# sshaoshuai/PointRCNN

Hardware: AMD Instinct MI355X
Metric: KITTI frames/sec, RPN inference end-to-end (16384 pts/frame, bs32 per GPU) (higher is better)
Workload: dtype f32 via split-bf16x6 MFMA (every fp32 operand cut exactly into 3 bf16 pieces, 6 bf16 MFMA products per fp32 product, fp32 accumulate: fp32-grade, measured error 2.9e-7 of sum|x||w| vs 3.0e-7 for the fp32-MFMA kernel; hoisted grouped layers on the split kernel too, unhoisted grouped first layers (xyz; 1 GPU; Full RPN PointNet++ backbone (4 SA-MSG + 4 FP) + cls/reg heads, tools/cfgs/default.yaml, 16384 pts/frame, batch 32 per GPU, random-init weights, eval-mode BN; frames_per_gpu=32, npoints=16384, parallelism=frames sharded, dp1, launch=hipGraph replay, streams=20, hw_queues=4, proposal_layer=normal, clouds=uniform, group_dedup=True, roi_dedup=True

## Files before the change

### include/prcnn_pointops.h

```cpp
#ifndef PRCNN_POINTOPS_H
#define PRCNN_POINTOPS_H

#include <stddef.h>
#include <stdint.h>

#ifdef __cplusplus
extern "C" {
#endif

typedef void* prcnn_stream_t;

#define PRCNN_OK 0
#define PRCNN_EINVAL (-1)
#define PRCNN_EHIP (-2)
#define PRCNN_EUNSUPPORTED (-3)

int prcnn_abi_version(void);
const char* prcnn_last_error(void);
const char* prcnn_build_id(void);


int prcnn_fps(const float* xyz, int B, int N, int npoint, float* tmp, int32_t* idx, prcnn_stream_t stream);

int prcnn_fps_status(void);
// ... 34 lines not shown
                       float* out, prcnn_stream_t stream);
int prcnn_three_interp_grad(const float* grad_out, const int32_t* idx, const float* weight, int B, int C, int n,
                            int m, float* grad_feat, float* workspace, prcnn_stream_t stream);


size_t prcnn_wpack_floats(int Nout, int K);
int prcnn_pack_weight(const float* w, int Nout, int K, int k_rot, float* wpack, prcnn_stream_t stream);

int prcnn_mlp_rows(const float* in, int ld_in, int64_t rows, int K, const float* wpack, const float* bias, int Nout,
                   int relu, float* out, int ld_out, int col_off, int pool_ns, const int32_t* rows_dev, int rows_unit,
                   const int32_t* seg_cnt, int seg_rows, prcnn_stream_t stream);

int prcnn_mlp_group(const float* xyz, const float* new_xyz, const int32_t* idx, const float* feat_cl, int ld_feat,
                    int B, int N, int M, int nsample, int C, const float* act_wx, const float* act_bias,
                    const float* wpack, const float* bias, int Nout, int relu, float* out, int ld_out, int col_off,
                    int pool_ns, const int32_t* groups_dev, prcnn_stream_t stream);

int prcnn_mlp_interp(const float* known_cl, int ld_known, const int32_t* idx3, const float* w3, const float* skip_cl,
                     int ld_skip, int B, int n, int m, int C2, int C1, const float* act_bias, const float* wpack,
                     const float* bias, int Nout, int relu, float* out, int ld_out, int col_off,
                     prcnn_stream_t stream);

int prcnn_mlp_rows_addinterp(const float* in, int ld_in, int K, const float* wpack, const float* bias, int Nout,
                             int relu, const float* y_cl, int ld_y, const int32_t* idx3, const float* w3, int B, int n,
                             int m, float* out, int ld_out, int col_off, prcnn_stream_t stream);

size_t prcnn_wsplit_bytes(int Nout, int K);
int prcnn_pack_weight_split(const float* w, int Nout, int K, int chain, void* wsplit, prcnn_stream_t stream);
int prcnn_mlp_rows_split(const float* in, int ld_in, int64_t rows, int K, const float* wpack, const void* wsplit, int terms,
                         const float* bias, int Nout, int relu, float* out, int ld_out, int col_off, int pool_ns,
                         const int32_t* rows_dev, int rows_unit, const int32_t* seg_cnt, int seg_rows, prcnn_stream_t stream);
int prcnn_mlp_chain_rows_split(const float* in, int ld_in, int64_t rows, int K, const void* const* wchain, const float* const* wpack,
                               const float* const* bias, const int* nout, const int* relu, int terms, float* out, int ld_out,
                               int col_off, prcnn_stream_t stream);
int prcnn_mlp_chain_interp_split(const float* known_cl, int ld_known, const int32_t* idx3, const float* w3, int B, int n, int m,
                                 int C2, const float* act_bias, const void* wchain, const float* wpack, const float* bias, int Nout,
                                 int relu, int terms, float* out, int ld_out, int col_off, prcnn_stream_t stream);
int prcnn_mlp_rows_addinterp_split(const float* in, int ld_in, int K, const float* wpack, const void* wsplit, int terms,
                                   const float* bias, int Nout, int relu, const float* y_cl, int ld_y, const int32_t* idx3,
                                   const float* w3, int B, int n, int m, float* out, int ld_out, int col_off,
                                   prcnn_stream_t stream);
int prcnn_mlp_group_split(const float* xyz, const float* new_xyz, const int32_t* idx, const float* feat_cl, int ld_feat, int B, int N,
                          int M, int nsample, int C, const float* act_wx, const float* act_bias, const float* wpack,
                          const void* wsplit, int terms, const float* bias, int Nout, int relu, float* out, int ld_out, int col_off,
                          int pool_ns, const int32_t* groups_dev, prcnn_stream_t stream);

int prcnn_mlp_chain_supported(int mode, int nlayers, const int* nout, int pool_ns);
int prcnn_mlp_chain_rows(const float* in, int ld_in, int64_t rows, int K, int nlayers, const float* const* wpack,
                         const float* const* bias, const int* nout, const int* relu, float* out, int ld_out,
                         int col_off, int pool_ns, const int32_t* seg_cnt, int seg_rows, prcnn_stream_t stream);
int prcnn_mlp_chain_group(const float* xyz, const float* new_xyz, const int32_t* idx, const float* feat_cl,
                          int ld_feat, int B, int N, int M, int nsample, int C, const float* act_wx,
                          const float* act_bias, int nlayers,
                          const float* const* wpack, const float* const* bias, const int* nout, const int* relu,
                          float* out, int ld_out, int col_off, int pool_ns, const int32_t* groups_dev, prcnn_stream_t stream);
int prcnn_mlp_chain_interp(const float* known_cl, int ld_known, const int32_t* idx3, const float* w3,
                           const float* skip_cl, int ld_skip, int B, int n, int m, int C2, int C1,
                           const float* act_bias, int nlayers, const float* const* wpack, const float* const* bias, const int* nout, const int* relu,
                           float* out, int ld_out, int col_off, prcnn_stream_t stream);

int prcnn_maxpool_rows(const float* in, int ld_in, int64_t rows_out, int ns, int C, float* out, int ld_out,
                       int col_off, prcnn_stream_t stream);

int prcnn_roipool3d(const float* xyz, const float* boxes3d, const float* feat, int B, int N, int M, int C, int S,
                    float* pooled, int32_t* empty, prcnn_stream_t stream);
size_t prcnn_roipool3d_work_bytes(int B, int N);
int prcnn_roipool3d_ws(const float* xyz, const float* boxes3d, const float* feat, int B, int N, int M, int C, int S, float* pooled,
                       int32_t* empty, void* work, size_t work_bytes, prcnn_stream_t stream);

int prcnn_pts_in_boxes3d(const float* pts, const float* boxes3d, int N, int M, int32_t* flags, prcnn_stream_t stream);
// ... 134 lines not shown
```

### pointrcnn_amd/_cabi.py

```python
import ctypes
import os

from . import build as _build

_P = ctypes.c_void_p
_I = ctypes.c_int
_F = ctypes.c_float
_L = ctypes.c_int64
_Z = ctypes.c_size_t
_D = ctypes.c_double



class TrainSrc(ctypes.Structure):
    _fields_ = [("mode", _I), ("rows", _L), ("K", _I),
                ("in_", _P), ("ld_in", _I), ("pro_scale", _P), ("pro_shift", _P),
                ("xyz", _P), ("new_xyz", _P), ("idx", _P), ("feat", _P), ("ld_feat", _I),
                ("B", _I), ("N", _I), ("M", _I), ("ns", _I), ("C", _I),
                ("known", _P), ("idx3", _P), ("w3", _P), ("skip", _P), ("ld_known", _I), ("ld_skip", _I),
                ("n", _I), ("m", _I), ("C2", _I), ("C1", _I),
                ("mult", _P), ("rows_dev", _P), ("norm_rows", _L), ("seg_off", _P), ("seg_cnt", _P), ("row_grp", _P), ("groups", _I)]


class TrainLayer(ctypes.Structure):
    _fields_ = [("Nout", _I), ("W", _P), ("gamma", _P), ("beta", _P), ("eps", _F), ("momentum", _F),
                ("running_mean", _P), ("running_var", _P), ("y", _P), ("cst", _P), ("ld_c", _I), ("wpack", _P), ("wpack_t", _P),
                ("dW", _P), ("dgamma", _P), ("dbeta", _P)]


REQUIRED_ABI = 9

SIGNATURES = {
    "prcnn_abi_version": (_I, []),
    "prcnn_last_error": (ctypes.c_char_p, []),
    "prcnn_build_id": (ctypes.c_char_p, []),
    "prcnn_fps": (_I, [_P, _I, _I, _I, _P, _P, _P]),
    "prcnn_fps_status": (_I, []),
    "prcnn_fps_order": (_I, [_P, _I, _I, _I, _I, _P, _P, _P]),
    "prcnn_fps_mode": (_I, [_P, _I, _I, _I, _I, _I, _P, _P, _P]),
    "prcnn_ball_query_arith": (_I, [_P, _P, _I, _I, _I, _F, _I, _I, _P, _P]),
    "prcnn_three_nn_arith": (_I, [_P, _P, _I, _I, _I, _I, _P, _P, _P]),
    "prcnn_rpn_labels": (_I, [_P, _P, _P, _I, _I, _I, _F, _P, _P, _P]),
    "prcnn_gt_aug_edit": (_I, [_P, _P, _P, _P, _P, _F, _P, _P, _P, _I, _I, _I, _I, _P, _P, _P, _P, _P]),
    "prcnn_host_pts_in_boxes3d": (_I, [_P, _P, _L, _L, _P]),
    "prcnn_host_roipool3d": (_I, [_P, _P, _P, _L, _L, _L, _L, _P, _P, _P]),
    "prcnn_gather": (_I, [_P, _P, _I, _I, _I, _I, _P, _P]),
    "prcnn_gather_grad": (_I, [_P, _P, _I, _I, _I, _I, _P, _P]),
    "prcnn_gather_rows": (_I, [_P, _I, _P, _I, _I, _I, _I, _P, _P]),
    "prcnn_ball_query": (_I, [_P, _P, _I, _I, _I, _F, _I, _P, _P]),
    "prcnn_ball_query2": (_I, [_P, _P, _I, _I, _I, _F, _I, _P, _F, _I, _P, _P]),
    "prcnn_group": (_I, [_P, _P, _I, _I, _I, _I, _I, _P, _P]),
    "prcnn_group_grad": (_I, [_P, _P, _I, _I, _I, _I, _I, _P, _P]),
    "prcnn_three_nn": (_I, [_P, _P, _I, _I, _I, _P, _P, _P, _P]),
    "prcnn_three_interp": (_I, [_P, _P, _P, _I, _I, _I, _I, _P, _P]),
    "prcnn_three_interp_grad": (_I, [_P, _P, _P, _I, _I, _I, _I, _P, _P, _P]),
    "prcnn_wpack_floats": (_Z, [_I, _I]),
    "prcnn_pack_weight": (_I, [_P, _I, _I, _I, _P, _P]),
    "prcnn_mlp_rows": (_I, [_P, _I, _L, _I, _P, _P, _I, _I, _P, _I, _I, _I, _P, _I, _P, _I, _P]),
    "prcnn_mlp_group": (_I, [_P, _P, _P, _P, _I, _I, _I, _I, _I, _I, _P, _P, _P, _P, _I, _I, _P, _I, _I, _I, _P, _P]),
    "prcnn_mlp_group_split": (_I, [_P, _P, _P, _P, _I, _I, _I, _I, _I, _I, _P, _P, _P, _P, _I, _P, _I, _I, _P, _I, _I, _I, _P, _P]),
    "prcnn_mlp_interp": (_I, [_P, _I, _P, _P, _P, _I, _I, _I, _I, _I, _I, _P, _P, _P, _I, _I, _P, _I, _I, _P]),
    "prcnn_mlp_rows_addinterp": (_I, [_P, _I, _I, _P, _P, _I, _I, _P, _I, _P, _P, _I, _I, _I, _P, _I, _I, _P]),
    "prcnn_wsplit_bytes": (_Z, [_I, _I]),
    "prcnn_pack_weight_split": (_I, [_P, _I, _I, _I, _P, _P]),
    "prcnn_mlp_chain_interp_split": (_I, [_P, _I, _P, _P, _I, _I, _I, _I, _P, _P, _P, _P, _I, _I, _I, _P, _I, _I, _P]),
    "prcnn_mlp_chain_rows_split": (_I, [_P, _I, _L, _I, _P, _P, _P, _P, _P, _I, _P, _I, _I, _P]),
    "prcnn_mlp_rows_split": (_I, [_P, _I, _L, _I, _P, _P, _I, _P, _I, _I, _P, _I, _I, _I, _P, _I, _P, _I, _P]),
    "prcnn_mlp_rows_addinterp_split": (_I, [_P, _I, _I, _P, _P, _I, _P, _I, _I, _P, _I, _P, _P, _I, _I, _I, _P, _I, _I, _P]),
    "prcnn_mlp_chain_supported": (_I, [_I, _I, _P, _I]),
    "prcnn_mlp_chain_rows": (_I, [_P, _I, _L, _I, _I, _P, _P, _P, _P, _P, _I, _I, _I, _P, _I, _P]),
    "prcnn_mlp_chain_group": (_I, [_P, _P, _P, _P, _I, _I, _I, _I, _I, _I, _P, _P, _I, _P, _P, _P, _P, _P, _I, _I, _I, _P, _P]),
    "prcnn_mlp_chain_interp": (_I, [_P, _I, _P, _P, _P, _I, _I, _I, _I, _I, _I, _P, _I, _P, _P, _P, _P, _P, _I, _I, _P]),
    "prcnn_maxpool_rows": (_I, [_P, _I, _L, _I, _I, _P, _I, _I, _P]),
    "prcnn_roipool3d": (_I, [_P, _P, _P, _I, _I, _I, _I, _I, _P, _P, _P]),
    "prcnn_roipool3d_work_bytes": (_Z, [_I, _I]),
    "prcnn_roipool3d_ws": (_I, [_P, _P, _P, _I, _I, _I, _I, _I, _P, _P, _P, _Z, _P]),
    "prcnn_pts_in_boxes3d": (_I, [_P, _P, _I, _I, _P, _P]),
    "prcnn_boxes_overlap_bev": (_I, [_P, _I, _P, _I, _P, _P]),
    "prcnn_boxes_iou_bev": (_I, [_P, _I, _P, _I, _P, _P]),
    "prcnn_nms_workspace_bytes": (_Z, [_I]),
    "prcnn_nms": (_I, [_P, _I, _F, _I, _I, _P, _P, _P, _Z, _P]),
    "prcnn_decode_bbox_target": (_I, [_P, _I, _P, ctypes.c_long, _I, _D, _D, _I, _P, _I, _I, _D, _D, _I, _I, _P, _P]),
    "prcnn_proposal_workspace_bytes": (_Z, [_I, _I, _I, _I]),
    "prcnn_proposal_layer": (_I, [_P, _P, _I, _I, _I, _F, _F, _F, _I, _I, _I, _I, _F, _I, _P, _P, _P, _P, _Z, _P]),
    "prcnn_nms_batched_workspace_bytes": (_Z, [_I, _I]),
    "prcnn_roipool3d_canonical": (_I, [_P, _P, _P, _P, _P, _P, _I, _I, _I, _I, _I, _I, _P, _I, _P, _I, _P, _P, _P]),
    "prcnn_roipool3d_canonical_ws": (_I, [_P, _P, _P, _P, _P, _P, _I, _I, _I, _I, _I, _I, _P, _I, _P, _I, _P, _P, _P, _Z, _P]),
    "prcnn_grid_bytes": (_Z, [_I, _I]),
    "prcnn_grid_build": (_I, [_P, _I, _I, _F, _I, _P, _Z, _P]),
    "prcnn_ball_query2_grid": (_I, [_P, _P, _P, _I, _I, _I, _F, _I, _P, _F, _I, _P, _P]),
    "prcnn_three_nn_grid": (_I, [_P, _P, _I, _I, _I, _P, _P, _P, _P]),
    "prcnn_rotate_iou_eval": (_I, [_P, _I, _P, _I, _I, _P, _P]),
    "prcnn_kitti_overlaps": (_I, [_I, _P, _P, _P, _P, _P, _I, _P, _P]),
    "prcnn_kitti_statistics": (_I, [_P, _P, _P, _P, _P, _P, _P, _P, _P, _P, _I, _I, _I, _D, _P, _I, _I, _I, _P, _P, _P]),
    "prcnn_group_compact": (_I, [_P, _P, _I, _I, _I, _I, _I, _P, _P, _P, _P, _P, _P, _P, _P, _P, _P, _P]),
    "prcnn_segmax_scatter": (_I, [_P, _I, _P, _P, _P, _P, _I, _I, _P, _I, _I, _P]),
    "prcnn_scatter_rows": (_I, [_P, _I, _P, _P, _I, _I, _P, _I, _I, _P]),
    "prcnn_scene_workspace_bytes": (_Z, [_L, _I]),
    "prcnn_scene_prepare": (_I, [_P, _P, _I, _L, _I, _P, _P, _P, _I, ctypes.c_uint32, _P, _P, _P, _P, _P, _P, _Z, _P]),
# ... 73 lines not shown
```

### pointrcnn_amd/csrc/cabi_common.hip

```cpp
#include "common.h"
#include <stdarg.h>

static thread_local char g_err[512] = "";

int prcnn_fail(int code, const char* fmt, ...) {
    va_list ap;
    va_start(ap, fmt);
    vsnprintf(g_err, sizeof(g_err), fmt, ap);
    va_end(ap);
    return code;
}

PRCNN_API const char* prcnn_last_error(void) { return g_err; }
PRCNN_API int prcnn_abi_version(void) { return 9; }

#ifndef PRCNN_BUILD_ID
#define PRCNN_BUILD_ID "PRCNN_BUILD_ID=unknown"
#endif
PRCNN_API const char* prcnn_build_id(void) { return &PRCNN_BUILD_ID[sizeof("PRCNN_BUILD_ID=") - 1]; }
```

### pointrcnn_amd/csrc/mlp.hip

```cpp
#include "common.h"
#include <stdlib.h>

#define MLP_BM 128
#define MLP_BN 64
#define MLP_BK 32
#define MLP_THREADS 256
#define MLP_ALD 36

typedef float f32x16 __attribute__((ext_vector_type(16)));

enum { MODE_PLAIN = 0, MODE_GROUP = 1, MODE_INTERP = 2 };

struct MlpParams {
    long rows;
    int K, KB, NB;
    const float* wpack;
    const float* bias;
    int Nout, relu;
    float* out;
    int ld_out, col_off, pool_ns;
    const float* in;
    int ld_in;
    const float* xyz;
    const float* new_xyz;
// ... 980 lines not shown
        bool bad = wave_has_nonfinite<2 * WNB>(reinterpret_cast<const f32x16 (&)[2 * WNB]>(acc));
        if (ADDY && addy_done) bad = __syncthreads_or(bad) != 0;
        if (bad && n_active) split_redo_f32<MODE, WNB>(P, acc, row0, wm, wn, nb0, lane);
        if (bad) addy_done = false;
    }
    layer_epilogue<MODE, WNB, ADDY>(P, acc, reinterpret_cast<float*>(Ls), nullptr, tid, row0, nb0, n_active, addy_done);
}

template <int MODE, int WNB, int TERMS, bool ADDY, bool LOOP>
__global__ __launch_bounds__(MLP_THREADS, 2) void mlp_layer_s_kernel(const MlpParams Pin) {
    MlpParams P = Pin;
    P.rows = effective_rows(Pin);
    __shared__ __attribute__((aligned(16))) unsigned char Ls[2 * 3 * SPL_PLANE];
    if constexpr (LOOP) {
        const long nbid = ((P.rows + MLP_BM - 1) / MLP_BM + 7) / 8 * 8 * P.wgm_cols;
        for (long bid = blockIdx.x; bid < nbid; bid += gridDim.x) {
            int tid;
            asm volatile("v_mov_b32 %0, %1" : "=v"(tid) : "v"(threadIdx.x));
            layer_s_tile<MODE, WNB, TERMS, ADDY>(P, bid, 0, tid, Ls);
            __syncthreads();
        }
    } else {
        layer_s_tile<MODE, WNB, TERMS, ADDY>(P, blockIdx.x, blockIdx.y, threadIdx.x, Ls);
    }
}

struct ChainParams {
    MlpParams a;
    const float* wpack1; const float* bias1; int KB1, N1, relu1;
    const float* wpack2; const float* bias2; int KB2, N2, relu2;
    int nlayers;
    int stack_split;
    const void* wsplit1;
};

#define CH_DPP_FMAX(v, ctrl) asm volatile("s_nop 1\n\tv_max_f32_dpp %0, %0, %0 " ctrl : "+v"(v))
#define CH_DPP_FMAX4(v, ctrl)                                                                                   \
    asm volatile("s_nop 1\n\tv_max_f32_dpp %0, %0, %0 " ctrl "\n\tv_max_f32_dpp %1, %1, %1 " ctrl               \
                 "\n\tv_max_f32_dpp %2, %2, %2 " ctrl "\n\tv_max_f32_dpp %3, %3, %3 " ctrl                       \
                 : "+v"(v[0]), "+v"(v[1]), "+v"(v[2]), "+v"(v[3]))

__device__ __forceinline__ float4 ldw(const float* __restrict__ wpack, int KB, int ob, int kb, int lane) {
    return ld4(wpack + (((long)ob * KB + kb) * 64 + lane) * 4);
}

template <int NB>
__device__ __forceinline__ void bias_act(f32x16 (&acc)[NB], const float* __restrict__ bias, int relu, int h) {
#pragma unroll
    for (int ob = 0; ob < NB; ob++)
#pragma unroll
        for (int q = 0; q < 4; q++) {
            float4 b = bias ? ld4(bias + ob * 32 + 8 * q + 4 * h) : make_float4(0.f, 0.f, 0.f, 0.f);
            float v0 = acc[ob][4 * q + 0] + b.x, v1 = acc[ob][4 * q + 1] + b.y;
            float v2 = acc[ob][4 * q + 2] + b.z, v3 = acc[ob][4 * q + 3] + b.w;
            if (relu) { v0 = fmaxf(v0, 0.f); v1 = fmaxf(v1, 0.f); v2 = fmaxf(v2, 0.f); v3 = fmaxf(v3, 0.f); }
            acc[ob][4 * q + 0] = v0; acc[ob][4 * q + 1] = v1; acc[ob][4 * q + 2] = v2; acc[ob][4 * q + 3] = v3;
        }
}

#define CH_WAVES 4
#define CH_STAGE_TILES 16
template <int NB> struct ChStage { static constexpr int G = CH_STAGE_TILES / NB; static constexpr int TPW = (G * NB + CH_WAVES - 1) / CH_WAVES; };

template <int NB>
__device__ __forceinline__ void stage_load(const float* __restrict__ wpack, int KB, int st, int wave, int lane, float4 (&r)[4]) {
    constexpr int G = ChStage<NB>::G;
// ... 830 lines not shown
        mt.w0[u] = w[0]; mt.w1[u] = w[1]; mt.w2[u] = w[2];
    }
}
__device__ __forceinline__ void coop_rows32(const MlpParams& P, long rw0, int g, int q, const CoopMeta<MODE_PLAIN>&, CoopRows32<MODE_PLAIN>& cr) {
#pragma unroll
    for (int u = 0; u < 4; u++) cr.o[u] = (unsigned)(min(rw0 + 8 * u + g, P.rows - 1) * (long)P.ld_in) + 4u * q;
}
__device__ __forceinline__ void coop_rows32(const MlpParams& P, long rw0, int g, int q, const CoopMeta<MODE_INTERP>& mt, CoopRows32<MODE_INTERP>& cr) {
#pragma unroll
    for (int u = 0; u < 4; u++) {
        const long r = min(rw0 + 8 * u + g, P.rows - 1);
        const long base = (r / P.n) * (long)P.m;
        cr.o0[u] = (unsigned)((base + mt.i0[u]) * (long)P.ld_known) + 4u * q;
        cr.o1[u] = (unsigned)((base + mt.i1[u]) * (long)P.ld_known) + 4u * q;
        cr.o2[u] = (unsigned)((base + mt.i2[u]) * (long)P.ld_known) + 4u * q;
        cr.w0[u] = mt.w0[u]; cr.w1[u] = mt.w1[u]; cr.w2[u] = mt.w2[u];
    }
}
__device__ __forceinline__ void coop_fetch32(const MlpParams& P, const CoopRows32<MODE_PLAIN>& cr, int c, CoopRaw<MODE_PLAIN>& v) {
#pragma unroll
    for (int u = 0; u < 4; u++) v.a[u] = ld4(P.in + cr.o[u] + 32 * c);
}
__device__ __forceinline__ void coop_fetch32(const MlpParams& P, const CoopRows32<MODE_INTERP>& cr, int c, CoopRaw<MODE_INTERP>& v) {
#pragma unroll
    for (int u = 0; u < 4; u++) {
        v.a[u] = ld4(P.known + cr.o0[u] + 32 * c); v.b[u] = ld4(P.known + cr.o1[u] + 32 * c); v.c[u] = ld4(P.known + cr.o2[u] + 32 * c);
    }
}
__device__ __forceinline__ float4 coop_finish32(const CoopRows32<MODE_PLAIN>&, const CoopRaw<MODE_PLAIN>& v, int u, float4) { return v.a[u]; }
__device__ __forceinline__ float4 coop_finish32(const CoopRows32<MODE_INTERP>& cr, const CoopRaw<MODE_INTERP>& v, int u, float4 b) {
    return interp_bias_relu4(cr.w0[u], cr.w1[u], cr.w2[u], v.a[u], v.b[u], v.c[u], b);
}

struct CoopTiles {
    long t;
    long step, end;
    long f, i, tpf, wx, WX, nframes;
    bool xcd;
};
__device__ __forceinline__ void coop_tiles_init(CoopTiles& it, const MlpParams& P, int wave) {
    const long ntiles = (P.rows + 31) / 32;
    it.xcd = P.xcd_tpf > 0 && (gridDim.x & 7) == 0;
    if (it.xcd) {
        it.tpf = 4L * P.xcd_tpf; it.nframes = ntiles / it.tpf;
        it.WX = (long)(gridDim.x >> 3) * CP_WAVES; it.wx = (long)(blockIdx.x >> 3) * CP_WAVES + wave;
        it.f = blockIdx.x & 7; it.i = it.wx;
        it.t = (it.i < it.tpf && it.f < it.nframes) ? it.f * it.tpf + it.i : -1;
    } else {
        it.step = (long)gridDim.x * CP_WAVES; it.end = ntiles;
        it.t = (long)blockIdx.x * CP_WAVES + wave;
        if (it.t >= it.end) it.t = -1;
    }
}
__device__ __forceinline__ long coop_tiles_next(CoopTiles& it) {
    if (it.t < 0) return -1;
    if (it.xcd) {
        it.i += it.WX;
        if (it.i >= it.tpf) { it.i = it.wx; it.f += 8; }
        it.t = (it.f < it.nframes) ? it.f * it.tpf + it.i : -1;
    } else {
        it.t += it.step;
        if (it.t >= it.end) it.t = -1;
    }
    return it.t;
}

template <int MODE, int NB1, int TERMS>
__global__ __launch_bounds__(CP_WAVES * 64, 1) void mlp_chain_p_kernel(const ChainParams Cin) {
    static_assert(NB1 == 0 || NB1 == 1, "one layer, or one layer + the single-channel output");
    constexpr int NB0 = 4, NST = 4;
    constexpr int RD = MODE == MODE_PLAIN ? 2 : 1;
    ChainParams C = Cin;
    C.a.rows = effective_rows(Cin.a);
    const MlpParams& P = C.a;
    const int tid = threadIdx.x, lane = tid & 63;
    const int wave = __builtin_amdgcn_readfirstlane(tid >> 6);
    const int h = lane >> 5, j = lane & 31, g = lane >> 3, q = lane & 7;

    extern __shared__ __attribute__((aligned(16))) unsigned char cp_lds[];
    uint4* Wl = reinterpret_cast<uint4*>(cp_lds);
    float* Tw = reinterpret_cast<float*>(cp_lds + (size_t)NST * SStage<NB0>::U4 * 16) + wave * 32 * CC_LD;
    float* s_bias = reinterpret_cast<float*>(cp_lds + (size_t)NST * SStage<NB0>::U4 * 16) + CP_WAVES * 32 * CC_LD;
    float* s_b = s_bias + 128;
    {
        const u32x4* img = reinterpret_cast<const u32x4*>(P.wsplit);
        for (int e = tid; e < NST * SStage<NB0>::U4; e += CP_WAVES * 64) reinterpret_cast<u32x4*>(Wl)[e] = img[e];
        if (tid < 128) { s_bias[tid] = P.bias ? P.bias[tid] : 0.f; s_b[tid] = MODE != MODE_PLAIN ? P.act_bias[tid] : 0.f; }
    }
    __syncthreads();
    const bool out1 = NB1 == 1;
    const bool coop_out = P.pool_ns == 0 && ((P.ld_out | P.col_off) % 4 == 0) && aligned16(P.out) && P.Nout % 4 == 0;

#ifdef MLP_TIMING
    unsigned long long tacc[8] = {0, 0, 0, 0, 0, 0, 0, 0}, tlast = __builtin_readcyclecounter();
#endif
    CoopTiles it;
    coop_tiles_init(it, P, wave);
    if (it.t < 0) return;
    long cur = it.t;
    CoopMeta<MODE> mt;
    CoopRows32<MODE> cr;
    CoopRaw<MODE> x[NST];
    coop_meta_fetch(P, cur * 32, g, mt);
    coop_rows32(P, cur * 32, g, q, mt, cr);
#pragma unroll
    for (int c = 0; c < RD; c++) coop_fetch32(P, cr, c, x[c]);
    MLP_T(0)

    while (cur >= 0) {
        const long rw0 = cur * 32;
        const long nxt = coop_tiles_next(it);
        const long nrw0 = (nxt >= 0 ? nxt : cur) * 32;
        CoopRows32<MODE> crn;
        f32x16 a0[NB0];
#pragma unroll
        for (int ob = 0; ob < NB0; ob++) a0[ob] = (f32x16){0};
#pragma unroll
        for (int st = 0; st < NST; st++) {
            if (st == 0) coop_meta_fetch(P, nrw0, g, mt);
            int qo = 4 * q;
            asm volatile("" : "+v"(qo));
            const float4 b4 = MODE != MODE_PLAIN ? ld4(s_b + 32 * st + qo) : make_float4(0.f, 0.f, 0.f, 0.f);
            if (MODE == MODE_PLAIN) {
                if (st + RD == NST) coop_rows32(P, nrw0, g, q, mt, crn);
                if (st + RD < NST) coop_fetch32(P, cr, st + RD, x[st + RD]);
                else coop_fetch32(P, crn, st + RD - NST, x[st + RD - NST]);
            }
#pragma unroll
            for (int u = 0; u < 4; u++) *reinterpret_cast<float4*>(Tw + (8 * u + g) * CC_LD + 4 * q) = coop_finish32(cr, x[st], u, b4);
            if (MODE != MODE_PLAIN) {
                if (st + RD == NST) coop_rows32(P, nrw0, g, q, mt, crn);
                if (st + RD < NST) coop_fetch32(P, cr, st + RD, x[st + RD]);
                else coop_fetch32(P, crn, st + RD - NST, x[st + RD - NST]);
            }
            MLP_T(1)
            __builtin_amdgcn_wave_barrier();
#pragma unroll
            for (int ksl = 0; ksl < 2; ksl++) {
                const float4 va = *reinterpret_cast<const float4*>(Tw + j * CC_LD + 16 * ksl + 4 * h);
                const float4 vb = *reinterpret_cast<const float4*>(Tw + j * CC_LD + 16 * ksl + 8 + 4 * h);
                const float v[8] = {va.x, va.y, va.z, va.w, vb.x, vb.y, vb.z, vb.w};
                bf16x8 bp[3];
                split8(v, bp);
                unsigned wo = (unsigned)(st * SStage<NB0>::U4 + lane) * 16u;
// ... 21 lines not shown
        cur = nxt;
        MLP_T(7)
#ifdef MLP_TIMING
        if (lane == 0 && wave == 0) atomicAdd(&g_mlp_t[8], 1ULL);
#endif
    }
#ifdef MLP_TIMING
    if (lane == 0 && wave == 0) for (int k = 0; k < 8; k++) atomicAdd(&g_mlp_t[k], tacc[k]);
#endif
}
template <int MODE, int NB1> static constexpr size_t chain_p_lds_bytes() {
    return (size_t)4 * SStage<4>::U4 * 16 + (size_t)CP_WAVES * 32 * CC_LD * 4 + 2 * 128 * 4;
}
static int chain_p_grid() {
    static const int cus = [] {
        int dev = 0, n = 0;
        if (hipGetDevice(&dev) != hipSuccess || hipDeviceGetAttribute(&n, hipDeviceAttributeMultiprocessorCount, dev) != hipSuccess || n <= 0) n = 256;
        return n & ~7;
    }();
    return cus > 0 ? cus : 8;
}
static bool chain_persist_on() {
    const char* e = getenv("PRCNN_CHAIN_PERSIST");
    return !(e && atoi(e) == 0);
}
template <int MODE, int NB1>
static int launch_chain_p(const ChainParams& C, hipStream_t s) {
    constexpr size_t lds = chain_p_lds_bytes<MODE, NB1>();
    static PrcnnLdsLimit attr;
    if (!attr.raise((const void*)mlp_chain_p_kernel<MODE, NB1, 6>, (int)lds))
        return prcnn_fail(PRCNN_EHIP, "prcnn_mlp_chain(persistent split): cannot raise the dynamic LDS limit");
    const long tiles = (C.a.rows + 31) / 32;
    const int grid = (int)min((long)chain_p_grid(), (tiles + CP_WAVES - 1) / CP_WAVES);
    hipLaunchKernelGGL((mlp_chain_p_kernel<MODE, NB1, 6>), dim3(grid), dim3(CP_WAVES * 64), lds, s, C);
    return PRCNN_OK;
}
static bool chain_coop_on() {
    const char* e = getenv("PRCNN_CHAIN_COOP");
    return !(e && atoi(e) == 0);
}
static bool chain_coop_forced() {
    const char* e = getenv("PRCNN_CHAIN_COOP");
    return e && atoi(e) == 2;
}

#define PERS_WAVES 8
template <int KB, int NB>
__device__ __forceinline__ void pers_load_layer(float* dst, const float* __restrict__ wpack, int wave, int lane) {
    for (int t = wave; t < KB * NB; t += PERS_WAVES) {
        const int kb = t / NB, ob = t - kb * NB;
        *reinterpret_cast<float4*>(dst + (t * 64 + lane) * 4) = ldw(wpack, KB, ob, kb, lane);
    }
}
template <int NBI, int NBO>
__device__ __forceinline__ void pers_layer(const f32x16 (&in)[NBI], f32x16 (&out)[NBO], const float* wl, int lane) {
#pragma unroll
    for (int ob = 0; ob < NBO; ob++) out[ob] = (f32x16){0};
#pragma unroll
    for (int kb = 0; kb < NBI * 4; kb++) {
        const int pb = kb / 4, q = kb % 4;
        float4 w[NBO];
#pragma unroll
        for (int ob = 0; ob < NBO; ob++) w[ob] = lds_w(wl, kb * NBO + ob, lane);
#pragma unroll
        for (int ob = 0; ob < NBO; ob++) out[ob] = __builtin_amdgcn_mfma_f32_32x32x2f32(w[ob].x, in[pb][4 * q + 0], out[ob], 0, 0, 0);
#pragma unroll
// ... 310 lines not shown
PRCNN_API size_t prcnn_wpack_floats(int Nout, int K) {
    if (Nout <= 0 || K <= 0) return 0;
    return (size_t)((Nout + 31) / 32) * ((K + 7) / 8) * 256;
}

PRCNN_API int prcnn_pack_weight(const float* w, int Nout, int K, int k_rot, float* wpack, prcnn_stream_t stream) {
    PRCNN_REQUIRE(w && wpack, "prcnn_pack_weight: null pointer");
    PRCNN_REQUIRE(Nout > 0 && K > 0 && k_rot >= 0 && k_rot <= K, "prcnn_pack_weight: bad shape Nout=%d K=%d k_rot=%d", Nout, K, k_rot);
    int KB = (K + 7) / 8, NB = (Nout + 31) / 32;
    long total = (long)NB * KB * 256;
    hipLaunchKernelGGL(pack_weight_kernel, dim3(prcnn_divup(total, 256)), dim3(256), 0, (hipStream_t)stream, w, Nout, K,
                       k_rot, KB, NB, wpack);
    PRCNN_LAUNCH_CHECK("prcnn_pack_weight");
    return PRCNN_OK;
}

PRCNN_API size_t prcnn_wsplit_bytes(int Nout, int K) {
    if (Nout <= 0 || K <= 0) return 0;
    return (size_t)((Nout + 31) / 32) * ((K + 15) / 16) * 3 * 1024;
}

PRCNN_API int prcnn_pack_weight_split(const float* w, int Nout, int K, int chain, void* wsplit, prcnn_stream_t stream) {
    PRCNN_REQUIRE(w && wsplit && aligned16(wsplit), "prcnn_pack_weight_split: null / misaligned pointer");
    PRCNN_REQUIRE(Nout > 0 && K > 0 && (chain == 0 || chain == 1), "prcnn_pack_weight_split: bad shape Nout=%d K=%d chain=%d", Nout, K, chain);
    const int KS = (K + 15) / 16, NB = (Nout + 31) / 32;
    hipLaunchKernelGGL(pack_weight_split_kernel, dim3(prcnn_divup((long)NB * KS * 64, 256)), dim3(256), 0, (hipStream_t)stream, w,
                       Nout, K, KS, NB, chain, reinterpret_cast<uint4*>(wsplit));
    PRCNN_LAUNCH_CHECK("prcnn_pack_weight_split");
    return PRCNN_OK;
}

PRCNN_API int prcnn_mlp_chain_rows_split(const float* in, int ld_in, int64_t rows, int K, const void* const* wchain, const float* const* wpack,
                                         const float* const* bias, const int* nout, const int* relu, int terms, float* out, int ld_out,
                                         int col_off, prcnn_stream_t stream) {
    PRCNN_REQUIRE(in && wchain && wpack && bias && nout && relu && out, "prcnn_mlp_chain_rows_split: null pointer");
    PRCNN_REQUIRE(terms == 3 || terms == 6, "prcnn_mlp_chain_rows_split: terms=%d (3 or 6)", terms);
    PRCNN_REQUIRE(wpack[0] && wpack[1] && aligned16(wpack[0]) && aligned16(wpack[1]), "prcnn_mlp_chain_rows_split: the fp32 pack images of both layers are needed (non-finite rows, single-channel output)");
    const float* wpack1 = wpack[1];
    const bool ok = K == 128 && nout[0] == 128 && (nout[1] == 1 || (nout[1] > 64 && nout[1] <= 128)) && aligned16(in) && ld_in % 4 == 0 &&
                    ld_in >= K && wchain[0] && (nout[1] == 1 || wchain[1] != nullptr);
    if (!ok) return PRCNN_EUNSUPPORTED;
    PRCNN_REQUIRE(ld_out >= col_off + nout[1], "prcnn_mlp_chain_rows_split: ld_out=%d < col_off+Nout", ld_out);
    if (rows == 0) return PRCNN_OK;
    ChainParams C = {};
    MlpParams& P = C.a;
    P.rows = rows; P.K = K; P.in = in; P.ld_in = ld_in; P.bias = bias[0]; P.Nout = nout[0]; P.relu = relu[0];
    P.out = out; P.ld_out = ld_out; P.col_off = col_off; P.rows_unit = 1;
    P.wsplit = wchain[0]; P.split_terms = terms; P.wpack = wpack[0];
    C.wsplit1 = wchain[1]; C.wpack1 = wpack1; C.bias1 = bias[1]; C.N1 = nout[1]; C.relu1 = relu[1]; C.KB1 = 16; C.nlayers = 2;
    const dim3 grid(prcnn_divup(rows, 128));
    const hipStream_t s = (hipStream_t)stream;
#define SCH_LAUNCH(NB1)                                                                                        \
    do {                                                                                                       \
         \
         \
        if (terms == 6 && chain_coop_forced()) hipLaunchKernelGGL((mlp_chain_c_kernel<MODE_PLAIN, NB1, 6>), grid, dim3(256), 0, s, C); \
        else if (terms == 6) hipLaunchKernelGGL((mlp_chain_s_kernel<MODE_PLAIN, NB1, 6>), grid, dim3(256), 0, s, C); \
        else hipLaunchKernelGGL((mlp_chain_s_kernel<MODE_PLAIN, NB1, 3>), grid, dim3(256), 0, s, C);            \
    } while (0)
    if (nout[1] == 1 && terms == 6 && chain_coop_on() && chain_persist_on() && (long)rows * ld_in < (1L << 30)) {
        const int rc = launch_chain_p<MODE_PLAIN, 1>(C, s);
        if (rc) return rc;
    } else if (nout[1] == 1) SCH_LAUNCH(1);
    else if (nout[1] <= 96) SCH_LAUNCH(3);
    else SCH_LAUNCH(4);
#undef SCH_LAUNCH
    PRCNN_LAUNCH_CHECK("prcnn_mlp_chain_rows_split");
    return PRCNN_OK;
}

PRCNN_API int prcnn_mlp_rows_split(const float* in, int ld_in, int64_t rows, int K, const float* wpack, const void* wsplit, int terms,
                                   const float* bias, int Nout, int relu, float* out, int ld_out, int col_off, int pool_ns,
                                   const int32_t* rows_dev, int rows_unit, const int32_t* seg_cnt, int seg_rows, prcnn_stream_t stream) {
    PRCNN_REQUIRE(in && wsplit, "prcnn_mlp_rows_split: null pointer");
    PRCNN_REQUIRE(ld_in >= K && ld_out >= col_off + Nout, "prcnn_mlp_rows_split: bad strides ld_in=%d K=%d ld_out=%d", ld_in, K, ld_out);
    PRCNN_REQUIRE(terms == 3 || terms == 6, "prcnn_mlp_rows_split: terms=%d (3 or 6)", terms);
    MlpParams P = {};
    P.rows = rows; P.K = K; P.wpack = wpack; P.bias = bias; P.Nout = Nout; P.relu = relu;
    P.out = out; P.ld_out = ld_out; P.col_off = col_off; P.pool_ns = pool_ns;
    P.in = in; P.ld_in = ld_in;
    P.vec_a = aligned16(in) && (ld_in % 4 == 0);
    P.rows_dev = rows_dev; P.rows_unit = rows_unit > 0 ? rows_unit : 1;
// ... 617 lines not shown
    C.a.rows = (long)B * M * nsample; C.a.K = C_ + 3;
    C.a.rows_dev = groups_dev; C.a.rows_unit = nsample;
    C.a.xyz = xyz; C.a.new_xyz = new_xyz; C.a.idx = idx; C.a.feat = feat_cl; C.a.ld_feat = ld_feat;
    C.a.N = N; C.a.M = M; C.a.ns = nsample; C.a.C = C_;
    C.a.vec_a = C_ > 0 && aligned16(feat_cl) && (ld_feat % 4 == 0);
    rc = set_group_act(C.a, act_wx, act_bias, C_);
    if (rc) return rc;
    return dispatch_chain(MODE_GROUP, C, (hipStream_t)stream);
}

PRCNN_API int prcnn_mlp_chain_interp(const float* known_cl, int ld_known, const int32_t* idx3, const float* w3,
                                     const float* skip_cl, int ld_skip, int B, int n, int m, int C2, int C1,
                                     const float* act_bias, int nlayers, const float* const* wpack, const float* const* bias,
                                     const int* nout, const int* relu, float* out, int ld_out, int col_off,
                                     prcnn_stream_t stream) {
    PRCNN_REQUIRE(known_cl && idx3 && w3 && (C1 == 0 || skip_cl), "prcnn_mlp_chain_interp: null pointer");
    PRCNN_REQUIRE(B >= 0 && n > 0 && m > 0 && C2 > 0 && C1 >= 0 && ld_known >= C2 && (C1 == 0 || ld_skip >= C1), "prcnn_mlp_chain_interp: bad shape");
    ChainParams C = {};
    int rc = fill_chain(C, nlayers, wpack, bias, nout, relu, out, ld_out, col_off, 0);
    if (rc) return rc;
    C.a.rows = (long)B * n; C.a.K = C2 + C1;
    C.a.known = known_cl; C.a.idx3 = idx3; C.a.w3 = w3; C.a.skip = skip_cl; C.a.ld_known = ld_known; C.a.ld_skip = ld_skip;
    C.a.n = n; C.a.m = m; C.a.C2 = C2; C.a.C1 = C1;
    C.a.vec_a = aligned16(known_cl) && (ld_known % 4 == 0);
    C.a.vec_b = C1 > 0 && aligned16(skip_cl) && (ld_skip % 4 == 0) && (C2 % 4 == 0);
    rc = set_interp_act(C.a, act_bias, C2, C1);
    if (rc) return rc;
    if (B % 8 == 0 && n % 128 == 0 && getenv("PRCNN_NO_XCD_ORDER") == nullptr) C.a.xcd_tpf = n / 128;
    return dispatch_chain(MODE_INTERP, C, (hipStream_t)stream);
}

PRCNN_API int prcnn_mlp_chain_interp_split(const float* known_cl, int ld_known, const int32_t* idx3, const float* w3, int B, int n,
                                           int m, int C2, const float* act_bias, const void* wchain, const float* wpack, const float* bias,
                                           int Nout, int relu, int terms, float* out, int ld_out, int col_off, prcnn_stream_t stream) {
    PRCNN_REQUIRE(known_cl && idx3 && w3 && act_bias && wchain && wpack && aligned16(wpack) && out, "prcnn_mlp_chain_interp_split: null / misaligned pointer");
    PRCNN_REQUIRE(terms == 3 || terms == 6, "prcnn_mlp_chain_interp_split: terms=%d (3 or 6)", terms);
    PRCNN_REQUIRE(B >= 0 && n > 0 && m > 0 && ld_known >= C2 && ld_out >= col_off + Nout, "prcnn_mlp_chain_interp_split: bad shape");
    if (!(C2 == 128 && Nout == 128 && aligned16(known_cl) && ld_known % 4 == 0 && aligned16(act_bias))) return PRCNN_EUNSUPPORTED;
    if (B == 0) return PRCNN_OK;
    ChainParams C = {};
    MlpParams& P = C.a;
    P.rows = (long)B * n; P.K = C2; P.bias = bias; P.Nout = Nout; P.relu = relu;
    P.out = out; P.ld_out = ld_out; P.col_off = col_off; P.rows_unit = 1;
    P.known = known_cl; P.idx3 = idx3; P.w3 = w3; P.ld_known = ld_known; P.n = n; P.m = m; P.C2 = C2; P.C1 = 0;
    P.vec_a = 1; P.act = 2; P.act_bias = act_bias;
    P.wsplit = wchain; P.split_terms = terms; P.wpack = wpack;
    C.nlayers = 1;
    if (B % 8 == 0 && n % 128 == 0 && getenv("PRCNN_NO_XCD_ORDER") == nullptr) P.xcd_tpf = n / 128;
    const dim3 grid(prcnn_divup(P.rows, 128));
    if (terms == 6 && chain_coop_on() && chain_persist_on() && (long)B * m * ld_known < (1L << 30)) {
        const int rc = launch_chain_p<MODE_INTERP, 0>(C, (hipStream_t)stream);
        if (rc) return rc;
    } else if (terms == 6 && chain_coop_on()) hipLaunchKernelGGL((mlp_chain_c_kernel<MODE_INTERP, 0, 6>), grid, dim3(256), 0, (hipStream_t)stream, C);
    else if (terms == 6) hipLaunchKernelGGL((mlp_chain_s_kernel<MODE_INTERP, 0, 6>), grid, dim3(256), 0, (hipStream_t)stream, C);
    else hipLaunchKernelGGL((mlp_chain_s_kernel<MODE_INTERP, 0, 3>), grid, dim3(256), 0, (hipStream_t)stream, C);
    PRCNN_LAUNCH_CHECK("prcnn_mlp_chain_interp_split");
    return PRCNN_OK;
}

#include "mlp_train.h"
```

### pointrcnn_amd/ops.py

```python
import ctypes
import os
import threading

import torch

from . import _cabi

_INT = torch.int32
_F32 = torch.float32
FPS_PRUNED = os.environ.get("PRCNN_FPS_PRUNED", "1") == "1"


def _stream():
    return torch.cuda.current_stream().cuda_stream


def _chk(t, name, dtype=_F32, ndim=None):
    if not isinstance(t, torch.Tensor):
        raise TypeError("%s must be a torch.Tensor" % name)
    if not t.is_cuda:
        raise RuntimeError("%s must be a CUDA(HIP) tensor: the HIP kernels are the only implementation" % name)
    if t.dtype != dtype:
        raise RuntimeError("%s must have dtype %s, got %s" % (name, dtype, t.dtype))
    if not t.is_contiguous():
# ... 203 lines not shown
    def __init__(self, weight, bias=None, relu=True, k_rot=0):
        _chk(weight, "weight", ndim=2)
        self.nout, self.k = weight.shape
        self.relu = bool(relu)
        L = _cabi.lib()
        self.wpack = torch.empty((L.prcnn_wpack_floats(self.nout, self.k),), dtype=_F32, device=weight.device)
        _cabi.check(L.prcnn_pack_weight(_p(weight), self.nout, self.k, k_rot, _p(self.wpack), _stream()),
                    "prcnn_pack_weight")
        self._w = weight if k_rot == 0 else None
        self._wsplit = None
        self.bias = None
        if bias is not None:
            _chk(bias.contiguous(), "bias", ndim=1)
            self.bias = torch.zeros(((self.nout + 31) // 32 * 32,), dtype=_F32, device=weight.device)
            self.bias[: self.nout] = bias


    def wsplit(self, chain=0):
        if self._wsplit is None:
            self._wsplit = {}
        if chain not in self._wsplit and self._w is not None and self.k % 32 == 0:
            L = _cabi.lib()
            img = torch.empty((L.prcnn_wsplit_bytes(self.nout, self.k),), dtype=torch.uint8, device=self._w.device)
            _cabi.check(L.prcnn_pack_weight_split(_p(self._w.contiguous()), self.nout, self.k, int(chain), _p(img), _stream()),
                        "prcnn_pack_weight_split")
            self._wsplit[chain] = img
        return self._wsplit.get(chain)


MLP_SPLIT_TERMS = int(os.environ.get("PRCNN_MLP_SPLIT", "6") or 0)
if MLP_SPLIT_TERMS not in (0, 3, 6):
    raise RuntimeError("PRCNN_MLP_SPLIT=%r: 6 (default) / 3 split-bf16 terms, 0 = fp32 MFMA" % os.environ.get("PRCNN_MLP_SPLIT"))

_MODE_ROWS, _MODE_GROUP, _MODE_INTERP = 0, 1, 2
_chain_ok = {}


def chain_supported(mode, layers, pool_ns=0):
    key = (mode, tuple(l.nout for l in layers), pool_ns)
    hit = _chain_ok.get(key)
    if hit is None:
        arr = (ctypes.c_int * len(layers))(*[l.nout for l in layers])
        hit = bool(_cabi.lib().prcnn_mlp_chain_supported(mode, len(layers), arr, pool_ns)) if 1 <= len(layers) <= 3 else False
        _chain_ok[key] = hit
    return hit


class _ChainArgs:

    def __init__(self, layers):
        n = len(layers)
        self.n = n
        self.layers = tuple(layers)
        self.wpack = (ctypes.c_void_p * n)(*[l.wpack.data_ptr() for l in layers])
        self.bias = (ctypes.c_void_p * n)(*[(l.bias.data_ptr() if l.bias is not None else None) for l in layers])
        self.nout = (ctypes.c_int * n)(*[l.nout for l in layers])
        self.relu = (ctypes.c_int * n)(*[int(l.relu) for l in layers])


def _chain_args(layers):
    key = tuple(id(l) for l in layers)
    hit = getattr(layers[0], "_chain_cache", None)
    if hit is None or hit[0] != key:
        hit = (key, _ChainArgs(layers))
        layers[0]._chain_cache = hit
    return hit[1]


def mlp_chain_rows(x, layers, out=None, pool_ns=0, seg=None):
    if x.stride(-1) != 1:
        raise RuntimeError("mlp_chain_rows: last dim must be contiguous")
    K = x.shape[-1]
    rows = x.numel() // K
    ld_in = _row_stride(x)
    rows_out = rows // pool_ns if pool_ns else rows
    buf, ld_out, col_off = _out_buf(out, rows_out, layers[-1], x.device)
    a = _chain_args(layers)
    seg_cnt, seg_rows = (None, 0) if seg is None else (seg[0], int(seg[1]))
    if (MLP_SPLIT_TERMS and not pool_ns and seg is None and a.n == 2 and K == 128 and layers[0].nout == 128
            and (layers[1].nout == 1 or 64 < layers[1].nout <= 128) and layers[0].wsplit(1) is not None and layers[1].wsplit(1) is not None):
        if getattr(a, "wchain", None) is None:
            a.wchain = (ctypes.c_void_p * 2)(layers[0].wsplit(1).data_ptr(), layers[1].wsplit(1).data_ptr())
        rc = _cabi.lib().prcnn_mlp_chain_rows_split(_p(x), ld_in, rows, K, a.wchain, a.wpack, a.bias, a.nout, a.relu,
                                                    MLP_SPLIT_TERMS, _p(buf), ld_out, col_off, _stream())
        if rc != _cabi.EUNSUPPORTED:
            _cabi.check(rc, "prcnn_mlp_chain_rows_split")
            return buf
    _cabi.check(_cabi.lib().prcnn_mlp_chain_rows(_p(x), ld_in, rows, K, a.n, a.wpack, a.bias, a.nout, a.relu, _p(buf),
                                                 ld_out, col_off, pool_ns, _p(seg_cnt), seg_rows, _stream()), "prcnn_mlp_chain_rows")
    return buf


def mlp_chain_group(xyz, new_xyz, idx, feat_cl, layers, out=None, pool_ns=0, act=None, groups_dev=None):
    B, N, _ = xyz.shape
    _, M, ns = idx.shape
    C = 0 if feat_cl is None else feat_cl.shape[-1]
    ld_feat = 0 if feat_cl is None else _row_stride(feat_cl)
    rows = B * M * ns
    rows_out = rows // pool_ns if pool_ns else rows
    buf, ld_out, col_off = _out_buf(out, rows_out, layers[-1], xyz.device)
    a = _chain_args(layers)
    awx, ab = (None, None) if act is None else act
    _cabi.check(_cabi.lib().prcnn_mlp_chain_group(_p(xyz), _p(new_xyz), _p(idx), _p(feat_cl), ld_feat, B, N, M, ns, C, _p(awx), _p(ab), a.n,
                                                  a.wpack, a.bias, a.nout, a.relu, _p(buf), ld_out, col_off, pool_ns,
                                                  _p(groups_dev), _stream()), "prcnn_mlp_chain_group")
    return buf


def mlp_chain_interp(known_cl, idx3, w3, skip_cl, layers, out=None, act_bias=None):
    B, m, C2 = known_cl.shape
    n = idx3.shape[1]
    C1 = 0 if skip_cl is None else skip_cl.shape[-1]
    ld_skip = 0 if skip_cl is None else _row_stride(skip_cl)
    buf, ld_out, col_off = _out_buf(out, B * n, layers[-1], known_cl.device)
    a = _chain_args(layers)
    if (MLP_SPLIT_TERMS and skip_cl is None and act_bias is not None and a.n == 1 and C2 == 128 and layers[0].nout == 128
            and layers[0].wsplit(1) is not None):
        l0 = layers[0]
        rc = _cabi.lib().prcnn_mlp_chain_interp_split(_p(known_cl), _row_stride(known_cl), _p(idx3), _p(w3), B, n, m, C2, _p(act_bias),
                                                      _p(l0.wsplit(1)), _p(l0.wpack), _p(l0.bias), l0.nout, int(l0.relu), MLP_SPLIT_TERMS, _p(buf),
                                                      ld_out, col_off, _stream())
        if rc != _cabi.EUNSUPPORTED:
            _cabi.check(rc, "prcnn_mlp_chain_interp_split")
            return buf
    _cabi.check(_cabi.lib().prcnn_mlp_chain_interp(_p(known_cl), _row_stride(known_cl), _p(idx3), _p(w3), _p(skip_cl), ld_skip,
                                                   B, n, m, C2, C1, _p(act_bias), a.n, a.wpack, a.bias, a.nout, a.relu, _p(buf),
                                                   ld_out, col_off, _stream()), "prcnn_mlp_chain_interp")
    return buf


def _row_stride(x):
    for size, stride in zip(reversed(x.shape[:-1]), reversed(x.stride()[:-1])):
        if size != 1:
            return stride
    return x.shape[-1]


def _out_buf(out, rows, lin, device):
    if out is None:
        return torch.empty((rows, lin.nout), dtype=_F32, device=device), lin.nout, 0
    buf, col_off = out
    return buf, _row_stride(buf), col_off


def mlp_rows(x, lin, out=None, pool_ns=0, rows_dev=None, rows_unit=1, seg=None):
    if x.stride(-1) != 1:
        raise RuntimeError("mlp_rows: last dim must be contiguous")
    K = x.shape[-1]
    rows = x.numel() // K
    ld_in = _row_stride(x)
    rows_out = rows // pool_ns if pool_ns else rows
    buf, ld_out, col_off = _out_buf(out, rows_out, lin, x.device)
    if MLP_SPLIT_TERMS and ld_in % 4 == 0 and (seg is None or (rows_dev is None and not pool_ns)) and lin.wsplit() is not None:
        _cabi.check(_cabi.lib().prcnn_mlp_rows_split(_p(x), ld_in, rows, K, _p(lin.wpack), _p(lin.wsplit()), MLP_SPLIT_TERMS,
# ... 434 lines not shown
```

Baseline: 13740 frames/s.

## Use atomic per-XCD tile claiming in persistent split MLP chain kernels

Replaces the static strided tile assignment in the persistent split-bf16 chain kernel with dynamic work stealing. Each wave claims tiles through atomic counters, one per XCD group, and moves on to other groups' counters once its home range is exhausted. The counters are zeroed before each launch, and the next claim is issued early to hide the atomic latency. This targets load imbalance and tail effects across waves, at the cost of per-tile atomics, an extra memset launch, and a small buffer allocated on every call.

```diff
diff --git a/include/prcnn_pointops.h b/include/prcnn_pointops.h
--- a/include/prcnn_pointops.h
+++ b/include/prcnn_pointops.h
@@ -90,10 +90,10 @@
                          const int32_t* rows_dev, int rows_unit, const int32_t* seg_cnt, int seg_rows, prcnn_stream_t stream);
 int prcnn_mlp_chain_rows_split(const float* in, int ld_in, int64_t rows, int K, const void* const* wchain, const float* const* wpack,
                                const float* const* bias, const int* nout, const int* relu, int terms, float* out, int ld_out,
-                               int col_off, prcnn_stream_t stream);
+                               int col_off, uint32_t* claim, prcnn_stream_t stream);
 int prcnn_mlp_chain_interp_split(const float* known_cl, int ld_known, const int32_t* idx3, const float* w3, int B, int n, int m,
                                  int C2, const float* act_bias, const void* wchain, const float* wpack, const float* bias, int Nout,
-                                 int relu, int terms, float* out, int ld_out, int col_off, prcnn_stream_t stream);
+                                 int relu, int terms, float* out, int ld_out, int col_off, uint32_t* claim, prcnn_stream_t stream);
 int prcnn_mlp_rows_addinterp_split(const float* in, int ld_in, int K, const float* wpack, const void* wsplit, int terms,
                                    const float* bias, int Nout, int relu, const float* y_cl, int ld_y, const int32_t* idx3,
                                    const float* w3, int B, int n, int m, float* out, int ld_out, int col_off,
diff --git a/pointrcnn_amd/_cabi.py b/pointrcnn_amd/_cabi.py
--- a/pointrcnn_amd/_cabi.py
+++ b/pointrcnn_amd/_cabi.py
@@ -28,7 +28,7 @@
                 ("dW", _P), ("dgamma", _P), ("dbeta", _P)]
 
 
-REQUIRED_ABI = 9
+REQUIRED_ABI = 10
 
 SIGNATURES = {
     "prcnn_abi_version": (_I, []),
@@ -63,8 +63,8 @@
     "prcnn_mlp_rows_addinterp": (_I, [_P, _I, _I, _P, _P, _I, _I, _P, _I, _P, _P, _I, _I, _I, _P, _I, _I, _P]),
     "prcnn_wsplit_bytes": (_Z, [_I, _I]),
     "prcnn_pack_weight_split": (_I, [_P, _I, _I, _I, _P, _P]),
-    "prcnn_mlp_chain_interp_split": (_I, [_P, _I, _P, _P, _I, _I, _I, _I, _P, _P, _P, _P, _I, _I, _I, _P, _I, _I, _P]),
-    "prcnn_mlp_chain_rows_split": (_I, [_P, _I, _L, _I, _P, _P, _P, _P, _P, _I, _P, _I, _I, _P]),
+    "prcnn_mlp_chain_interp_split": (_I, [_P, _I, _P, _P, _I, _I, _I, _I, _P, _P, _P, _P, _I, _I, _I, _P, _I, _I, _P, _P]),
+    "prcnn_mlp_chain_rows_split": (_I, [_P, _I, _L, _I, _P, _P, _P, _P, _P, _I, _P, _I, _I, _P, _P]),
     "prcnn_mlp_rows_split": (_I, [_P, _I, _L, _I, _P, _P, _I, _P, _I, _I, _P, _I, _I, _I, _P, _I, _P, _I, _P]),
     "prcnn_mlp_rows_addinterp_split": (_I, [_P, _I, _I, _P, _P, _I, _P, _I, _I, _P, _I, _P, _P, _I, _I, _I, _P, _I, _I, _P]),
     "prcnn_mlp_chain_supported": (_I, [_I, _I, _P, _I]),
diff --git a/pointrcnn_amd/csrc/cabi_common.hip b/pointrcnn_amd/csrc/cabi_common.hip
--- a/pointrcnn_amd/csrc/cabi_common.hip
+++ b/pointrcnn_amd/csrc/cabi_common.hip
@@ -12,7 +12,7 @@
 }
 
 PRCNN_API const char* prcnn_last_error(void) { return g_err; }
-PRCNN_API int prcnn_abi_version(void) { return 9; }
+PRCNN_API int prcnn_abi_version(void) { return 10; }
 
 #ifndef PRCNN_BUILD_ID
 #define PRCNN_BUILD_ID "PRCNN_BUILD_ID=unknown"
diff --git a/pointrcnn_amd/csrc/mlp.hip b/pointrcnn_amd/csrc/mlp.hip
--- a/pointrcnn_amd/csrc/mlp.hip
+++ b/pointrcnn_amd/csrc/mlp.hip
@@ -1036,6 +1036,7 @@
     int nlayers;
     int stack_split;
     const void* wsplit1;
+    unsigned* claim;
 };
 
 #define CH_DPP_FMAX(v, ctrl) asm volatile("s_nop 1\n\tv_max_f32_dpp %0, %0, %0 " ctrl : "+v"(v))
@@ -1932,15 +1933,50 @@
     return interp_bias_relu4(cr.w0[u], cr.w1[u], cr.w2[u], v.a[u], v.b[u], v.c[u], b);
 }
 
+#define CP_CLAIM_WORDS 512
 struct CoopTiles {
     long t;
     long step, end;
     long f, i, tpf, wx, WX, nframes;
     bool xcd;
+    unsigned* ctr;
+    int home, gk;
+    unsigned raw;
 };
-__device__ __forceinline__ void coop_tiles_init(CoopTiles& it, const MlpParams& P, int wave) {
+__device__ __forceinline__ void claim_issue(CoopTiles& it, int lane) {
+    unsigned* c = it.ctr + 64 * ((it.home + it.gk) & 7);
+    unsigned k = 0;
+    if (lane == 0) k = atomicAdd(c, 1u);
+    it.raw = k;
+}
+__device__ __forceinline__ long claim_take(CoopTiles& it, int lane) {
+    for (;;) {
+        const long k = (long)__builtin_amdgcn_readfirstlane(it.raw);
+        const int gx = (it.home + it.gk) & 7;
+        if (!it.xcd) {
+            const long lo = it.end * gx / 8, hi = it.end * (gx + 1) / 8;
+            if (lo + k < hi) return lo + k;
+        } else {
+            const long nfr = gx < it.nframes ? (it.nframes - 1 - gx) / 8 + 1 : 0;
+            if (k < nfr * it.tpf) return (gx + 8 * (k / it.tpf)) * it.tpf + k % it.tpf;
+        }
+        if (++it.gk == 8) return -1;
+        claim_issue(it, lane);
+    }
+}
+__device__ __forceinline__ void coop_tiles_init(CoopTiles& it, const MlpParams& P, int wave, unsigned* ctr, int lane) {
     const long ntiles = (P.rows + 31) / 32;
     it.xcd = P.xcd_tpf > 0 && (gridDim.x & 7) == 0;
+    it.ctr = ctr;
+    if (ctr) {
+        it.end = ntiles;
+        it.tpf = 4L * P.xcd_tpf; it.nframes = it.xcd ? ntiles / it.tpf : 0;
+        it.home = blockIdx.x & 7; it.gk = 0;
+        claim_issue(it, lane);
+        it.t = claim_take(it, lane);
+        if (it.t >= 0) claim_issue(it, lane);
+        return;
+    }
     if (it.xcd) {
         it.tpf = 4L * P.xcd_tpf; it.nframes = ntiles / it.tpf;
         it.WX = (long)(gridDim.x >> 3) * CP_WAVES; it.wx = (long)(blockIdx.x >> 3) * CP_WAVES + wave;
@@ -1952,8 +1988,13 @@
         if (it.t >= it.end) it.t = -1;
     }
 }
-__device__ __forceinline__ long coop_tiles_next(CoopTiles& it) {
+__device__ __forceinline__ long coop_tiles_next(CoopTiles& it, int lane) {
     if (it.t < 0) return -1;
+    if (it.ctr) {
+        it.t = claim_take(it, lane);
+        if (it.t >= 0) claim_issue(it, lane);
+        return it.t;
+    }
     if (it.xcd) {
         it.i += it.WX;
         if (it.i >= it.tpf) { it.i = it.wx; it.f += 8; }
@@ -1995,7 +2036,7 @@
     unsigned long long tacc[8] = {0, 0, 0, 0, 0, 0, 0, 0}, tlast = __builtin_readcyclecounter();
 #endif
     CoopTiles it;
-    coop_tiles_init(it, P, wave);
+    coop_tiles_init(it, P, wave, C.claim, lane);
     if (it.t < 0) return;
     long cur = it.t;
     CoopMeta<MODE> mt;
@@ -2009,7 +2050,7 @@
 
     while (cur >= 0) {
         const long rw0 = cur * 32;
-        const long nxt = coop_tiles_next(it);
+        const long nxt = coop_tiles_next(it, lane);
         const long nrw0 = (nxt >= 0 ? nxt : cur) * 32;
         CoopRows32<MODE> crn;
         f32x16 a0[NB0];
@@ -2097,6 +2138,8 @@
         return prcnn_fail(PRCNN_EHIP, "prcnn_mlp_chain(persistent split): cannot raise the dynamic LDS limit");
     const long tiles = (C.a.rows + 31) / 32;
     const int grid = (int)min((long)chain_p_grid(), (tiles + CP_WAVES - 1) / CP_WAVES);
+    if (C.claim && prcnn_fill_words(C.claim, 0u, CP_CLAIM_WORDS, s) != hipSuccess)
+        return prcnn_fail(PRCNN_EHIP, "prcnn_mlp_chain(persistent split): clearing the tile counters failed");
     hipLaunchKernelGGL((mlp_chain_p_kernel<MODE, NB1, 6>), dim3(grid), dim3(CP_WAVES * 64), lds, s, C);
     return PRCNN_OK;
 }
@@ -2473,7 +2516,7 @@
 
 PRCNN_API int prcnn_mlp_chain_rows_split(const float* in, int ld_in, int64_t rows, int K, const void* const* wchain, const float* const* wpack,
                                          const float* const* bias, const int* nout, const int* relu, int terms, float* out, int ld_out,
-                                         int col_off, prcnn_stream_t stream) {
+                                         int col_off, uint32_t* claim, prcnn_stream_t stream) {
     PRCNN_REQUIRE(in && wchain && wpack && bias && nout && relu && out, "prcnn_mlp_chain_rows_split: null pointer");
     PRCNN_REQUIRE(terms == 3 || terms == 6, "prcnn_mlp_chain_rows_split: terms=%d (3 or 6)", terms);
     PRCNN_REQUIRE(wpack[0] && wpack[1] && aligned16(wpack[0]) && aligned16(wpack[1]), "prcnn_mlp_chain_rows_split: the fp32 pack images of both layers are needed (non-finite rows, single-channel output)");
@@ -2489,6 +2532,7 @@
     P.out = out; P.ld_out = ld_out; P.col_off = col_off; P.rows_unit = 1;
     P.wsplit = wchain[0]; P.split_terms = terms; P.wpack = wpack[0];
     C.wsplit1 = wchain[1]; C.wpack1 = wpack1; C.bias1 = bias[1]; C.N1 = nout[1]; C.relu1 = relu[1]; C.KB1 = 16; C.nlayers = 2;
+    C.claim = claim;
     const dim3 grid(prcnn_divup(rows, 128));
     const hipStream_t s = (hipStream_t)stream;
 #define SCH_LAUNCH(NB1)                                                                                        \
@@ -3172,7 +3216,8 @@
 
 PRCNN_API int prcnn_mlp_chain_interp_split(const float* known_cl, int ld_known, const int32_t* idx3, const float* w3, int B, int n,
                                            int m, int C2, const float* act_bias, const void* wchain, const float* wpack, const float* bias,
-                                           int Nout, int relu, int terms, float* out, int ld_out, int col_off, prcnn_stream_t stream) {
+                                           int Nout, int relu, int terms, float* out, int ld_out, int col_off, uint32_t* claim,
+                                           prcnn_stream_t stream) {
     PRCNN_REQUIRE(known_cl && idx3 && w3 && act_bias && wchain && wpack && aligned16(wpack) && out, "prcnn_mlp_chain_interp_split: null / misaligned pointer");
     PRCNN_REQUIRE(terms == 3 || terms == 6, "prcnn_mlp_chain_interp_split: terms=%d (3 or 6)", terms);
     PRCNN_REQUIRE(B >= 0 && n > 0 && m > 0 && ld_known >= C2 && ld_out >= col_off + Nout, "prcnn_mlp_chain_interp_split: bad shape");
@@ -3186,6 +3231,7 @@
     P.vec_a = 1; P.act = 2; P.act_bias = act_bias;
     P.wsplit = wchain; P.split_terms = terms; P.wpack = wpack;
     C.nlayers = 1;
+    C.claim = claim;
     if (B % 8 == 0 && n % 128 == 0 && getenv("PRCNN_NO_XCD_ORDER") == nullptr) P.xcd_tpf = n / 128;
     const dim3 grid(prcnn_divup(P.rows, 128));
     if (terms == 6 && chain_coop_on() && chain_persist_on() && (long)B * m * ld_known < (1L << 30)) {
diff --git a/pointrcnn_amd/ops.py b/pointrcnn_amd/ops.py
--- a/pointrcnn_amd/ops.py
+++ b/pointrcnn_amd/ops.py
@@ -259,6 +259,12 @@
 if MLP_SPLIT_TERMS not in (0, 3, 6):
     raise RuntimeError("PRCNN_MLP_SPLIT=%r: 6 (default) / 3 split-bf16 terms, 0 = fp32 MFMA" % os.environ.get("PRCNN_MLP_SPLIT"))
 
+TILE_CLAIM = os.environ.get("PRCNN_TILE_CLAIM", "1") != "0"
+
+
+def _claim_words(device):
+    return torch.empty(512, dtype=torch.int32, device=device) if TILE_CLAIM else None
+
 _MODE_ROWS, _MODE_GROUP, _MODE_INTERP = 0, 1, 2
 _chain_ok = {}
 
@@ -308,8 +314,9 @@
             and (layers[1].nout == 1 or 64 < layers[1].nout <= 128) and layers[0].wsplit(1) is not None and layers[1].wsplit(1) is not None):
         if getattr(a, "wchain", None) is None:
             a.wchain = (ctypes.c_void_p * 2)(layers[0].wsplit(1).data_ptr(), layers[1].wsplit(1).data_ptr())
+        claim = _claim_words(x.device) if layers[1].nout == 1 else None
         rc = _cabi.lib().prcnn_mlp_chain_rows_split(_p(x), ld_in, rows, K, a.wchain, a.wpack, a.bias, a.nout, a.relu,
-                                                    MLP_SPLIT_TERMS, _p(buf), ld_out, col_off, _stream())
+                                                    MLP_SPLIT_TERMS, _p(buf), ld_out, col_off, _p(claim), _stream())
         if rc != _cabi.EUNSUPPORTED:
             _cabi.check(rc, "prcnn_mlp_chain_rows_split")
             return buf
@@ -344,9 +351,10 @@
     if (MLP_SPLIT_TERMS and skip_cl is None and act_bias is not None and a.n == 1 and C2 == 128 and layers[0].nout == 128
             and layers[0].wsplit(1) is not None):
         l0 = layers[0]
+        claim = _claim_words(known_cl.device)
         rc = _cabi.lib().prcnn_mlp_chain_interp_split(_p(known_cl), _row_stride(known_cl), _p(idx3), _p(w3), B, n, m, C2, _p(act_bias),
                                                       _p(l0.wsplit(1)), _p(l0.wpack), _p(l0.bias), l0.nout, int(l0.relu), MLP_SPLIT_TERMS, _p(buf),
-                                                      ld_out, col_off, _stream())
+                                                      ld_out, col_off, _p(claim), _stream())
         if rc != _cabi.EUNSUPPORTED:
             _cabi.check(rc, "prcnn_mlp_chain_interp_split")
             return buf
```

Result: no change. 13870 frames/s (median of 6 runs) (+0.9%).
